# langtech-bsc/quantool

Measured on AMD Instinct MI355X. Metric: quantized weights/sec (GPTQ int4, Llama-3-8B, 512 calib samples), higher is better.
Workload: dtype f32

## Files before the change

include/quantool_amd.h:

```cpp
#ifndef QUANTOOL_AMD_H
#define QUANTOOL_AMD_H

#include <stddef.h>
#include <stdint.h>

#ifdef __cplusplus
extern "C" {
#endif

typedef void* qt_stream_t;

enum qt_status {
    QT_OK = 0,
    QT_ERR_INVALID = -1,
    QT_ERR_NOT_PD = -2,
    QT_ERR_WORKSPACE = -3,
    QT_ERR_HIP = -4,
    QT_ERR_UNSUPPORTED = -5
};

enum qt_dtype { QT_F32 = 0, QT_BF16 = 1, QT_F16 = 2 };

int qt_version(void);
const char* qt_last_error(void);
// ... 73 lines not shown
int qt_awq_weight_mean_accumulate(const void* W, int w_dtype, int R, int K, int64_t ldw, int group_size,
                                  float* w_sum, void* workspace, size_t workspace_bytes,
                                  qt_stream_t stream);
int qt_awq_scales(const float* x_abs_sum, int64_t n_tokens, const float* w_sum, int64_t n_rows, int K,
                  int n_grid, int duo_scaling, float* scales, qt_stream_t stream);
int qt_symmetrize_lower(float* G, int K, qt_stream_t stream);
size_t qt_awq_loss_workspace_bytes(int R, int K);
int qt_awq_loss(const void* W, int w_dtype, int R, int K, int64_t ldw, const float* s, int group_size,
                int symmetric, int num_bits, const float* Gfull, int64_t n_tokens, int exact, float weight,
                int accumulate, float* loss_out, void* workspace, size_t workspace_bytes, qt_stream_t stream);
size_t qt_awq_losses_workspace_bytes(int R, int K, int n_grid);
int qt_awq_losses(const void* W, int w_dtype, int R, int K, int64_t ldw, const float* scales, int n_grid,
                  int group_size, int symmetric, int num_bits, const float* Gfull, int64_t n_tokens, float weight,
                  int accumulate, float* losses, void* workspace, size_t workspace_bytes, qt_stream_t stream);
int qt_argmin_f32(const float* values, int n, int32_t* index_out, qt_stream_t stream);
int qt_awq_pseudo_quantize(const void* W, int w_dtype, int R, int K, int64_t ldw, const float* s, int group_size,
                           int symmetric, int num_bits, void* out, int64_t ldo, qt_stream_t stream);
int qt_scale_columns(const void* W, int w_dtype, int R, int K, int64_t ldw, const float* s, int divide,
                     void* out, int64_t ldo, qt_stream_t stream);
int qt_rtn_quantize(const void* W, int w_dtype, int R, int K, int64_t ldw, const float* scale,
                    const float* zp, int G, int group_size, int num_bits, int8_t* Qt, qt_stream_t stream);

size_t qt_col_absmax_workspace_bytes(int R, int K);
int qt_col_absmax_accumulate(const void* W, int w_dtype, int R, int K, int64_t ldw, float* wmax,
                             void* workspace, size_t workspace_bytes, qt_stream_t stream);
int qt_smoothquant_scales(const float* cmin, const float* cmax, const float* wmax, int K, float alpha,
                          float* s, qt_stream_t stream);

size_t qt_sgemm_tn_f32_workspace_bytes(int M, int N);
int qt_sgemm_tn_f32(const float* A, int64_t lda, const float* B, int64_t ldb, const float* Cin,
                    int64_t ldcin, float* Cout, int64_t ldcout, int M, int N, int kdim, int skip_zero_k,
                    int mode, int allow_split_k, void* workspace, size_t workspace_bytes, qt_stream_t stream);

int qt_xtx_tile_table_check(int K, int* n_tiles_out, int* chunk_panels_out, int* round_panels_out);

size_t qt_xtx_dot_workspace_bytes(int64_t n_tokens, int K);
int qt_xtx_dot(const void* X, int x_dtype, int64_t n_tokens, int K, int64_t ldx, const float* H, double scale,
               float* out, int accumulate, void* workspace, size_t workspace_bytes, qt_stream_t stream);

size_t qt_gemm3_tn_f32_workspace_bytes(int M, int N, int k);
int qt_gemm3_tn_f32(const float* A, int64_t lda, const float* B, int64_t ldb, float* C, int64_t ldc, int M,
                    int N, int k, int kind, void* workspace, size_t workspace_bytes, qt_stream_t stream);
int qt_gemm3_tn_f32_ex(const float* A, int64_t lda, const float* B, int64_t ldb, float* C, int64_t ldc, int M, int N,
                       int k, int kind, int tri, int tight, int batch, int64_t bsA, int64_t bsB, int64_t bsC,
                       void* workspace, size_t workspace_bytes, qt_stream_t stream);

int qt_gemm3_tn_f16x2(const float* A, int64_t lda, const float* B, int64_t ldb, float* C, int64_t ldc, int M, int N,
                      int k, int kind, int tri, int tight, int batch, int64_t bsA, int64_t bsB, int64_t bsC,
                      const float* bound_a, const float* bound_b, void* workspace, size_t workspace_bytes,
                      qt_stream_t stream);

int qt_gemm3_plan_check(int Tm, int Tn, int c_end, int tri, int* n_items_out, int* n_slabs_out, int* longest_out);
int qt_chol_g3_plan_check(int K, int merged, int min_chunks, long long* counts_out);
enum qt_act { QT_ACT_SILU = 0 };
#define QT_I8_MID_MAX_M 128
#define QT_I8_MID_K_UNIT 128
#define QT_I8_RING_K_UNIT 128
#define QT_I8_RING_SLOTS 8
#define QT_I8_RING_LEAD 6
#define QT_I8_RING_W4_K_UNIT 128
#define QT_I8_RING_W4_SLOTS 8
#define QT_I8_RING_W4_LEAD 6
#define QT_SPLITK_I8_K_UNIT 128
#define QT_SPLITK_I8_MAX_SPLITS 32
#define QT_SPLITK_I8_MIN_K_TILES 4
#define QT_MOE_I8_WIDE_K_UNIT 128
#define QT_MOE_I8_WIDE_TILE_ROWS 128
#define QT_MOE_I8_WIDE_MAX_E 4096
enum qt_weight_format { QT_W_INT8 = 0, QT_W_INT4_PACKED = 1 };
int qt_quantize_tokens_i8(const void* X, int x_dtype, int64_t M, int K, int64_t ldx, const int32_t* col_perm,
                          int symmetric, int8_t* Xq, float* s_x, int32_t* zp_x, qt_stream_t stream);
int qt_act_mul_quantize_i8(const void* gate, int64_t ldg, const void* up, int64_t ldu, int x_dtype, int64_t M, int K,
                           int act, const int32_t* col_perm, int symmetric, int8_t* Xq, float* s_x, int32_t* zp_x,
                           void* H, int64_t ldh, qt_stream_t stream);
int qt_rmsnorm_quantize_i8(const void* X, int64_t ldx, const void* weight, int x_dtype, int64_t M, int K, float eps,
                           const int32_t* col_perm, int symmetric, int8_t* Xq, float* s_x, int32_t* zp_x,
                           void* Y, int64_t ldy, float* rstd, qt_stream_t stream);
int qt_gemm_i8(const int8_t* Xq, int64_t M, int K, const void* Wq, int w_format, int N, const float* s_x,
               const int32_t* zp_x, const float* s_w, int G, const int32_t* wsum, const void* bias, void* Y,
               int out_dtype, int64_t ldy, qt_stream_t stream);
int qt_gemm_i8_skinny(const int8_t* Xq, int M, int K, const void* Wq, int w_format, int N, const float* s_x,
                      const int32_t* zp_x, const float* s_w, int G, const int32_t* wsum, const void* bias, void* Y,
                      int out_dtype, int64_t ldy, qt_stream_t stream);
int qt_gemm_i8_ring(const int8_t* Xq, int64_t M, int K, const void* Wq, int w_format, int N, const float* s_x,
                    const int32_t* zp_x, const float* s_w, int G, const int32_t* wsum, const void* bias, void* Y,
                    int out_dtype, int64_t ldy, qt_stream_t stream);
int qt_gemm_i8_ring_w4(const int8_t* Xq, int64_t M, int K, const void* Wq, int w_format, int N, const float* s_x,
                       const int32_t* zp_x, const float* s_w, int G, const int32_t* wsum, const void* bias, void* Y,
                       int out_dtype, int64_t ldy, qt_stream_t stream);
int qt_gemm_i8_mid(const int8_t* Xq, int64_t M, int K, const void* Wq, int w_format, int N, const float* s_x,
                   const int32_t* zp_x, const float* s_w, int G, const int32_t* wsum, const void* bias, void* Y,
                   int out_dtype, int64_t ldy, qt_stream_t stream);
int qt_splitk_gemm_i8_plan(int64_t M, int N, int K, int cus, int splits_requested, int* splits,
                           size_t* workspace_size);
int qt_splitk_gemm_i8_range(int k_tiles, int splits, int s, int* t0, int* t1);
int qt_splitk_gemm_i8(const int8_t* Xq, int64_t M, int K, const void* Wq, int w_format, int N, const float* s_x,
                      const int32_t* zp_x, const float* s_w, int G, const int32_t* wsum, const void* bias, void* Y,
                      int out_dtype, int64_t ldy, int splits, void* workspace, size_t workspace_size,
                      qt_stream_t stream);

int qt_moe_route(const void* top_k_index, int index_is_int64, int64_t T, int k, int E, int32_t* offsets,
                 int32_t* src_token, int32_t* src_slot, int32_t* row_of, qt_stream_t stream);
int qt_gemm_i8_grouped(const int8_t* Xq, int K, const int32_t* row_idx, int64_t R, const int32_t* offsets, int E,
                       const void* Wq, int w_format, int N, const float* s_x, const int32_t* zp_x, const float* s_w,
                       int G, const int32_t* wsum, void* Y, int out_dtype, int64_t ldy, qt_stream_t stream);
int qt_gemm_i8_skinny_grouped(const int8_t* Xq, int K, const int32_t* row_idx, int64_t R, const int32_t* offsets,
// ... 66 lines not shown
```

quantool_amd/csrc/cholesky.hip:

```cpp
#include <stdlib.h>
#include <string.h>

#include <map>
#include <tuple>
#include <vector>

#include "chol_layout.h"
#include "common.h"
#include "gemm3_tn.h"
#include "sgemm_tn.h"

namespace {

static_assert(CHOL_CHUNK_ROWS == G3_CHUNK_ROWS, "chol_layout.h counts k chunks as gemm3_tn.h cuts them");
static int chol_block_env(const char* name) {
    const char* e = getenv(name);
    if (!e) return 0;
    int x = atoi(e) / 128 * 128;
    return x < 128 ? 128 : (x > NBO_MAX ? NBO_MAX : x);
}
struct G3Step {
    int n_items = 0, n_red = 0;
    size_t item_off = 0, red_off = 0;
};
struct CholG3Plan {
    bool any = false;
    std::vector<G3Step> fac, inv;
    std::vector<G3Step> row;
    char* blob = nullptr;
    size_t blob_bytes = 0;
    int max_slabs = 0;
    bool any_row = false;
};

static int chol_g3_min_chunks() {
    const char* on = getenv("QT_CHOL_G3");
    if (on && atoi(on) == 0) return 0;
    const char* e = getenv("QT_CHOL_G3_MIN_CHUNKS");
    const int x = e ? atoi(e) : 64;
    return x < 1 ? 1 : x;
}

static int chol_g3_target_items(int K) {
    const char* e = getenv("QT_G3_TARGET_ITEMS");
    if (e && atoi(e) > 0) return atoi(e);
    return K < 8192 ? 96 : 256;
}

enum { CHOL_TWO_PHASE = 0, CHOL_WALK = 1, CHOL_WALK_MERGED = 2 };
static int chol_merge_mode() {
    const char* e = getenv("QT_CHOL_MERGE");
    if (!e) return CHOL_WALK_MERGED;
    if (strcmp(e, "order") == 0) return CHOL_WALK;
    return atoi(e) != 0 ? CHOL_WALK_MERGED : CHOL_TWO_PHASE;
}

static void chol_g3_build(int K, int NBO, int NBI, int min_chunks, int target_items, bool merged, CholG3Plan& pl,
// ... 445 lines not shown
        for (int r = 0; r < 16; ++r) zb[r] = 0.0f;
#pragma unroll
        for (int r = 0; r < 16; ++r) {
            const int k = (r & 3) + 8 * (r >> 2) + 4 * h;
            const float av = D32[(b * 32 + k) * 32 + l31];
            zb = __builtin_amdgcn_mfma_f32_32x32x2f32(av, acc[b][r], zb, 0, 0, 0);
        }
        acc[b] = zb;
#pragma unroll
        for (int a = b + 1; a < 4; ++a) {
#pragma unroll
            for (int r = 0; r < 16; ++r) {
                const int k = (r & 3) + 8 * (r >> 2) + 4 * h;
                const float av = -Rs[(32 * b + k) * NB + 32 * a + l31];
                acc[a] = __builtin_amdgcn_mfma_f32_32x32x2f32(av, zb[r], acc[a], 0, 0, 0);
            }
        }
    }
    float* Dinv = Dinv_all + (size_t)blk * NB * NB;
    float* Yd = Y + (size_t)(blk * NB) * ldy + blk * NB;
#pragma unroll
    for (int a = 0; a < 4; ++a)
#pragma unroll
        for (int r = 0; r < 16; ++r) {
            const int row = 32 * a + (r & 3) + 8 * (r >> 2) + 4 * h;
            const bool in = row < n && col < n;
            const float z = (in && row >= col) ? acc[a][r] : 0.0f;
            Dinv[col * NB + row] = z;
            if (in) Yd[(size_t)row * ldy + col] = z;
        }
}

__global__ __launch_bounds__(256) void transpose_lower_block_kernel(const float* __restrict__ Y, int64_t ldy, int w,
                                                                    float* __restrict__ XT, int ldx, int64_t bsY,
                                                                    int64_t bsXT) {
    if (blockIdx.z) {
        Y += (size_t)blockIdx.z * bsY;
        XT += (size_t)blockIdx.z * bsXT;
    }
    __shared__ float tile[32][33];
    const int bx = blockIdx.x * 32, by = blockIdx.y * 32;
    const int tx = threadIdx.x & 31, ty = threadIdx.x >> 5;
    for (int r = ty; r < 32; r += 8) {
        const int m = bx + r, k = by + tx;
        tile[r][tx] = (m < w && k < w && k <= m) ? Y[(size_t)m * ldy + k] : 0.0f;
    }
    __syncthreads();
    for (int r = ty; r < 32; r += 8) {
        const int k = by + r, m = bx + tx;
        if (k < w && m < w) XT[(size_t)k * ldx + m] = tile[tx][r];
    }
}

__global__ __launch_bounds__(256) void flat_reverse_lower_to_upper_kernel(float* __restrict__ U, int K, int64_t bsU) {
    U += (size_t)blockIdx.z * bsU;
    const int j = blockIdx.x * blockDim.x + threadIdx.x;
    const int i = blockIdx.y;
    if (j >= K || j < i) return;
    const size_t e = (size_t)i * K + j;
    const size_t pe = (size_t)(K - 1 - i) * K + (K - 1 - j);
    if (i == j) {
        if (e <= pe) {
            const float t = U[e];
            U[e] = U[pe];
            U[pe] = t;
        }
    } else {
        U[e] = U[pe];
        U[pe] = 0.0f;
    }
}

__global__ __launch_bounds__(256) void identity_if_failed_kernel(float* __restrict__ U, int K,
                                                                 const int32_t* __restrict__ info, int64_t bsU) {
    if (info[blockIdx.z] == 0) return;
    U += (size_t)blockIdx.z * bsU;
    for (int i = blockIdx.x; i < K; i += gridDim.x)
        for (int j = threadIdx.x; j < K; j += blockDim.x) U[(size_t)i * K + j] = (i == j) ? 1.0f : 0.0f;
}

__global__ __launch_bounds__(256) void chol_scales_kernel(const float* __restrict__ A, int64_t bsA, int K,
                                                          const float* __restrict__ min_eig_lb, int32_t* __restrict__ e,
                                                          int32_t* __restrict__ info) {
    __shared__ float red[256];
    const int b = blockIdx.x, nprob = gridDim.x;
    const float* Ab = A + (size_t)b * bsA;
    float m = 0.0f;
    for (int i = threadIdx.x; i < K; i += 256) m = fmaxf(m, Ab[(size_t)i * K + i]);
    red[threadIdx.x] = m;
    __syncthreads();
    for (int s = 128; s > 0; s >>= 1) {
        if ((int)threadIdx.x < s) red[threadIdx.x] = fmaxf(red[threadIdx.x], red[threadIdx.x + s]);
        __syncthreads();
    }
    if (threadIdx.x == 0) {
        auto clampe = [](float t) { return (int)fminf(fmaxf(t, (float)-G3_E_MAX), (float)G3_E_MAX); };
        const float d = red[0], lb = min_eig_lb[b];
        e[b] = (d > 0.0f && d < 3.0e38f) ? clampe(3.0f - ceilf(0.5f * log2f(d))) : 0;
        if (lb > 0.0f && lb < 3.0e38f) {
            e[nprob + b] = clampe(3.0f - ceilf(-0.5f * log2f(lb)));
        } else {
            e[nprob + b] = 0;
            info[b] = K + 1;
        }
    }
}

}


static CholLayout chol_layout(int K, const CholG3Plan* g3) { return CholLayout(K, g3->any, g3->max_slabs); }

extern "C" size_t qt_cholesky_inverse_upper_batched_workspace_bytes(int K, int n_problems) {
    if (K <= 0 || n_problems <= 0) return 0;
    int nbo_, nbi_;
    const CholG3Plan* g3 = chol_blocks(K, nbo_, nbi_);
    return chol_layout(K, g3).batch_bytes(n_problems, g3->blob_bytes);
}

extern "C" size_t qt_cholesky_inverse_upper_workspace_bytes(int K) {
    return qt_cholesky_inverse_upper_batched_workspace_bytes(K, 1);
}

constexpr size_t INV_LDS = (size_t)(NB * LDT + NB * LDP) * sizeof(float);
constexpr size_t POTF2_LDS = (size_t)(NB * LDA + 4 * 32 * 32) * sizeof(float);
constexpr size_t RD_LDS = RD_STRIDE * sizeof(float);

struct CholCtx {
    float *A, *Y;
    int K, nprob, NBO, NBI;
    int64_t sA, sY, sW;
    float *T, *TI, *XT, *Rd, *Dinv, *split_ws;
    size_t split_ws_bytes;
    unsigned short *Rpl, *Ypl;
    int64_t plane_stride;
    float* g3_slabs;
    char* g3_tab;
    const CholG3Plan* g3;
    const CholG3Plan* tab;
    int planes;
    int merge_mode;
    int32_t *info, *eR, *eY;
    int prio;
    hipStream_t stream;
};

static int chol_resolve(CholCtx& c, const float* min_eig_lb) {
    bool f16x2 = min_eig_lb != nullptr;
    if (const char* e = getenv("QT_CHOL_PLANES")) {
        if (strcmp(e, "bf16x3") == 0) f16x2 = false;
        else if (strcmp(e, "f16x2") == 0) {
            QT_CHECK_ARG(min_eig_lb, "qt_cholesky_inverse_upper: QT_CHOL_PLANES=f16x2 needs a bound on lambda_min (the _bounded entry points)");
        } else {
            QT_CHECK_ARG(false, "qt_cholesky_inverse_upper: QT_CHOL_PLANES=%s (bf16x3 | f16x2)", e);
        }
    }
    c.g3 = chol_blocks(c.K, c.NBO, c.NBI);
    c.planes = (f16x2 && c.g3->any) ? G3_F16X2 : G3_BF16X3;
    c.merge_mode = (c.g3->any && c.NBO == c.NBI) ? chol_merge_mode() : CHOL_TWO_PHASE;
    c.tab = c.g3;
    if (c.merge_mode == CHOL_WALK_MERGED) {
        c.tab = chol_g3_plan(c.K, c.NBO, c.NBI, true);
        if (!c.tab->any || !c.tab->any_row || c.tab->max_slabs > c.g3->max_slabs || c.tab->blob_bytes > c.g3->blob_bytes) {
            c.tab = c.g3;
            c.merge_mode = CHOL_TWO_PHASE;
        }
    }
    return QT_OK;
}

enum CholHome { IN_A, IN_Y, IN_WS };
struct CholOperand { float* p; int64_t ld; CholHome home; };
static int64_t chol_stride(const CholCtx& c, CholHome h) { return h == IN_A ? c.sA : h == IN_Y ? c.sY : c.sW; }

static SgemmArgs chol_sgemm_args(const CholCtx& c, CholOperand A, CholOperand B, CholOperand C, int M, int N, int kdim,
                                 int k_mode, int mode, bool offer_split) {
    SgemmArgs g;
    g.A = A.p; g.lda = A.ld;
    g.B = B.p; g.ldb = B.ld;
    g.Cin = mode == SG_MODE_SUB ? C.p : nullptr; g.ldcin = mode == SG_MODE_SUB ? C.ld : 0;
    g.Cout = C.p; g.ldcout = C.ld;
    g.M = M; g.N = N; g.kdim = kdim; g.k_mode = k_mode; g.mode = mode;
    g.split_ws = offer_split ? c.split_ws : nullptr; g.split_ws_bytes = offer_split ? c.split_ws_bytes : 0;
    g.batch = c.nprob;
    g.bsA = chol_stride(c, A.home); g.bsB = chol_stride(c, B.home); g.bsCin = g.bsCout = chol_stride(c, C.home);
    g.bs_split = c.sW;
    return g;
}

static int g3_row(const CholCtx& c, const G3Step& st, const unsigned short* Bplanes, int col_a0, int col_b0, int M, int N,
                  float* C, CholHome c_home, int mode, bool second = false) {
    G3Args a;
    a.Apl = c.Rpl; a.Bpl = Bplanes; a.plane_stride = c.plane_stride; a.ld = c.K;
    a.rowA0 = a.rowB0 = 0; a.colA0 = col_a0; a.colB0 = col_b0; a.colmax = c.K;
    a.M = M; a.N = N; a.C = C; a.ldc = c.K; a.mode = mode;
    a.slabs = c.g3_slabs;
    a.items = (const G3Item*)(c.g3_tab + st.item_off); a.n_items = st.n_items;
    a.red = (const G3Red*)(c.g3_tab + st.red_off); a.n_red = st.n_red;
    a.batch = c.nprob;
    a.bsApl = a.bsBpl = c.sW * 2;
    a.bsC = chol_stride(c, c_home); a.bsSlabs = c.sW;
    if (c.planes == G3_F16X2) {
        a.planes = G3_F16X2; a.eA = c.eR; a.eB = Bplanes == c.Rpl ? c.eR : c.eY;
    }
    if (second) {
        a.Bpl1 = c.Ypl; a.colB01 = 0; a.eB1 = c.eY;
        a.C1 = c.TI; a.ldc1 = c.K; a.bsC1 = c.sW; a.mode1 = G3_SET;
        a.N1 = col_a0;
// ... 35 lines not shown
        }
    }
    const int rem = K - J1;
    if (c.g3->any) {
        if (rem > 0) {
            float* RJ = A + (size_t)J0 * K + J0;
            unsigned short* pl = c.Rpl + (size_t)J0 * K + J0;
            int rc = c.planes == G3_F16X2
                         ? qt_split2h_launch(RJ, K, J1 - J0, K - J0, pl, K, c.plane_stride, 0, 0, 0, c.eR, c.stream, nprob, c.sA, c.sW * 2)
                         : qt_split3_launch(RJ, K, J1 - J0, K - J0, pl, K, c.plane_stride, 0, 0, 0, c.stream, nprob, c.sA, c.sW * 2);
            if (rc) return rc;
        }
    } else if (rem > 0) {
        const CholOperand RJ = {A + (size_t)J0 * K + J1, K, IN_A};
        SgemmArgs g = chol_sgemm_args(c, RJ, RJ, {A + (size_t)J1 * K + J1, K, IN_A}, rem, rem, J1 - J0, SG_K_FULL, SG_MODE_SUB, false);
        g.upper_only = 1;
        int rc = qt_sgemm_tn(g, c.stream);
        if (rc) return rc;
    }
    return QT_OK;
}

static int trinv(const CholCtx& c, int blk0, int n) {
    const char* e = getenv("QT_CHOL_TRINV");
    if (e && strcmp(e, "div") == 0)
        hipLaunchKernelGGL(trinv_batched_kernel, dim3(n, c.nprob), dim3(NB), INV_LDS, c.stream, (const float*)c.Rd, c.K, c.Dinv,
                           c.Y, (int64_t)c.K, c.sW, c.sY, blk0);
    else
        hipLaunchKernelGGL(trinv_mfma_kernel, dim3(n, c.nprob), dim3(256), RD_LDS, c.stream, (const float*)c.Rd, c.K, c.Dinv,
                           c.Y, (int64_t)c.K, c.sW, c.sY, blk0);
    QT_LAUNCH_CHECK();
    return QT_OK;
}

static int inv_product(const CholCtx& c, const BlockRow& I) {
    const int K = c.K, I0 = I.J0;
    if (I0 == 0) return QT_OK;
    if (c.g3->any && c.tab->inv[I.Jb].n_items > 0) return g3_row(c, c.tab->inv[I.Jb], c.Ypl, I0, 0, I.rows(), I0, c.TI, IN_WS, G3_SET);
    return qt_sgemm_tn(chol_sgemm_args(c, {c.A + I0, K, IN_A}, {c.Y, K, IN_Y}, {c.TI, K, IN_WS}, I.rows(), I0, I0, SG_K_FROM_N0,
                                       SG_MODE_SET, true),
                       c.stream);
}

static int split_row(const CholCtx& c, const BlockRow& I) {
    const int K = c.K, I0 = I.J0;
    if (!c.g3->any || I.J1 >= K) return QT_OK;
    if (c.planes == G3_F16X2)
        return qt_split2h_launch(c.Y + (size_t)I0 * K, K, I.rows(), I.J1, c.Ypl + (size_t)I0 * K, K, c.plane_stride, 1, I0, 0, c.eY,
                                 c.stream, c.nprob, c.sY, c.sW * 2);
    return qt_split3_launch(c.Y + (size_t)I0 * K, K, I.rows(), I.J1, c.Ypl + (size_t)I0 * K, K, c.plane_stride, 1, I0, 0, c.stream,
                            c.nprob, c.sY, c.sW * 2);
}

static int inv_row(const CholCtx& c, const BlockRow& I) {
    const int K = c.K, I0 = I.J0, I1 = I.J1, Wi = I.rows();
    float* Y = c.Y;
    for (int i0 = I0 + NB; i0 < I1; i0 += NB) {
        const int i = i0 / NB, nbi = (K - i0 < NB) ? K - i0 : NB;
        const CholOperand Yi = {Y + (size_t)i0 * K + I0, K, IN_Y}, Tp = {c.T, K, IN_WS};
        int rc = qt_sgemm_tn(chol_sgemm_args(c, {c.A + (size_t)I0 * K + i0, K, IN_A}, {Y + (size_t)I0 * K + I0, K, IN_Y}, Tp, nbi,
                                             i0 - I0, i0 - I0, SG_K_FROM_N0, SG_MODE_SET, false),
                             c.stream);
        if (rc) return rc;
        rc = qt_sgemm_tn(chol_sgemm_args(c, {c.Dinv + (size_t)i * NB * NB, NB, IN_WS}, Tp, Yi, nbi, i0 - I0, nbi, SG_K_FULL,
                                         SG_MODE_NEG, false),
                         c.stream);
        if (rc) return rc;
    }
    if (I0 == 0) return split_row(c, I);
    hipLaunchKernelGGL(transpose_lower_block_kernel, dim3((Wi + 31) / 32, (Wi + 31) / 32, c.nprob), dim3(256), 0, c.stream,
                       (const float*)(Y + (size_t)I0 * K + I0), (int64_t)K, Wi, c.XT, NBO_MAX, c.sY, c.sW);
    QT_LAUNCH_CHECK();
    int rc = qt_sgemm_tn(chol_sgemm_args(c, {c.XT, NBO_MAX, IN_WS}, {c.TI, K, IN_WS}, {Y + (size_t)I0 * K, K, IN_Y}, Wi, I0, Wi,
                                         SG_K_FULL, SG_MODE_NEG, false),
                         c.stream);
    if (rc) return rc;
    return split_row(c, I);
}

static int chol_run_two_phase(const CholCtx& c) {
    for (BlockRow J(c.K, c.NBO); J; ++J) {
        int rc = fac_product(c, J);
        if (!rc) rc = fac_panels(c, J);
        if (rc) return rc;
    }
    int rc = trinv(c, 0, (c.K + NB - 1) / NB);
    if (rc) return rc;
    for (BlockRow I(c.K, c.NBI); I; ++I) {
        rc = inv_product(c, I);
        if (!rc) rc = inv_row(c, I);
        if (rc) return rc;
    }
    return QT_OK;
}

static int chol_run_walk(const CholCtx& c) {
    for (BlockRow J(c.K, c.NBO); J; ++J) {
        int rc;
        if (c.merge_mode == CHOL_WALK_MERGED && c.tab->row[J.Jb].n_items > 0) {
            rc = g3_row(c, c.tab->row[J.Jb], c.Rpl, J.J0, J.J0, J.rows(), c.K - J.J0, c.A + (size_t)J.J0 * c.K + J.J0, IN_A, G3_SUB,
                        true);
        } else {
            rc = fac_product(c, J);
            if (!rc) rc = inv_product(c, J);
        }
        if (!rc) rc = fac_panels(c, J);
        if (!rc) rc = trinv(c, J.J0 / NB, (J.rows() + NB - 1) / NB);
        if (!rc) rc = inv_row(c, J);
        if (rc) return rc;
    }
    return QT_OK;
}

static hipError_t chol_lds_attrs() {
    static QtOncePerDevice lds_attr;
    return lds_attr.run([] {
        const auto attr = hipFuncAttributeMaxDynamicSharedMemorySize;
        hipError_t e = hipFuncSetAttribute((const void*)potf2_kernel, attr, (int)POTF2_LDS);
        if (e == hipSuccess) e = hipFuncSetAttribute((const void*)trsm_rt_kernel, attr, (int)RD_LDS);
        if (e == hipSuccess) e = hipFuncSetAttribute((const void*)trinv_batched_kernel, attr, (int)INV_LDS);
        if (e == hipSuccess) e = hipFuncSetAttribute((const void*)trinv_mfma_kernel, attr, (int)RD_LDS);
        return e;
    });
}

static int chol_run(float* A, int64_t strideA, int K, float* U, int64_t strideU, int32_t* info, int nprob, void* workspace,
                    size_t workspace_bytes, hipStream_t stream, const float* min_eig_lb = nullptr) {
    CholCtx c = {};
    c.A = A; c.Y = U; c.K = K; c.nprob = nprob; c.info = info; c.stream = stream;
    if (int rc = chol_resolve(c, min_eig_lb)) return rc;
    const CholLayout L = chol_layout(K, c.g3);
    const size_t need = L.batch_bytes(nprob, c.g3->blob_bytes);
    if (!workspace || workspace_bytes < need) {
        qt_set_error("qt_cholesky_inverse_upper: workspace %zu < required %zu", workspace_bytes, need);
        return QT_ERR_WORKSPACE;
    }
    char* ws = (char*)qt_align_up((size_t)workspace, 256);
    c.sW = (int64_t)(L.bytes() / 4); c.sA = nprob > 1 ? strideA : 0; c.sY = nprob > 1 ? strideU : 0;
    c.T = (float*)(ws + L.T); c.TI = (float*)(ws + L.TI); c.XT = (float*)(ws + L.XT);
    c.Rd = (float*)(ws + L.Rd); c.Dinv = (float*)(ws + L.Dinv);
    c.split_ws = (float*)(ws + L.split); c.split_ws_bytes = L.split_bytes;
    c.plane_stride = (int64_t)K * K;
    if (c.g3->any) {
        c.Rpl = (unsigned short*)(ws + L.Rpl); c.Ypl = (unsigned short*)(ws + L.Ypl);
        c.g3_slabs = (float*)(ws + L.slabs); c.g3_tab = ws + L.tables(nprob);
        QT_HIP(hipMemcpyAsync(c.g3_tab, c.tab->blob, c.tab->blob_bytes, hipMemcpyHostToDevice, stream));
    }
    static_assert(2 * SG_MAX_BATCH * sizeof(int32_t) <= (size_t)NB * NB * 2, "the exponents fit the smallest third plane");
    c.eR = c.planes == G3_F16X2 ? (int32_t*)(c.Rpl + 2 * c.plane_stride) : nullptr;
    c.eY = c.planes == G3_F16X2 ? c.eR + nprob : nullptr;
    QT_HIP(chol_lds_attrs());
    QT_HIP(hipMemsetAsync(info, 0, sizeof(int32_t) * nprob, stream));
    c.prio = qt_chain_prio();
    if (c.planes == G3_F16X2) {
        hipLaunchKernelGGL(chol_scales_kernel, dim3(nprob), dim3(256), 0, stream, (const float*)A, c.sA, K, min_eig_lb, c.eR, info);
        QT_LAUNCH_CHECK();
    }
    if (int rc = c.merge_mode == CHOL_TWO_PHASE ? chol_run_two_phase(c) : chol_run_walk(c)) return rc;
    hipLaunchKernelGGL(flat_reverse_lower_to_upper_kernel, dim3((K + 255) / 256, K, nprob), dim3(256), 0, stream, U, K, c.sY);
    QT_LAUNCH_CHECK();
    hipLaunchKernelGGL(identity_if_failed_kernel, dim3(K < 1024 ? K : 1024, 1, nprob), dim3(256), 0, stream, U, K,
                       (const int32_t*)info, c.sY);
    QT_LAUNCH_CHECK();
    return QT_OK;
}

static int chol_check_batch(const char* fn, bool ptrs, int K, int n_problems, int64_t strideA, int64_t strideU) {
    QT_CHECK_ARG(K > 0 && ptrs && n_problems >= 1 && n_problems <= SG_MAX_BATCH, "%s: bad arguments (1 <= n_problems <= %d)", fn,
                 SG_MAX_BATCH);
    QT_CHECK_ARG(n_problems == 1 || (strideA >= (int64_t)K * K && strideU >= (int64_t)K * K && strideA % 4 == 0 && strideU % 4 == 0),
                 "%s: strides must be multiples of 4 elements and >= K*K", fn);
    return QT_OK;
}

extern "C" int qt_cholesky_inverse_upper(float* A, int K, float* U, int32_t* info, void* workspace,
                                         size_t workspace_bytes, qt_stream_t stream_) {
    QT_CHECK_ARG(K > 0 && A && U && info, "qt_cholesky_inverse_upper: bad arguments");
    return chol_run(A, 0, K, U, 0, info, 1, workspace, workspace_bytes, (hipStream_t)stream_);
}

extern "C" int qt_cholesky_inverse_upper_batched(float* A, int64_t strideA, int K, float* U, int64_t strideU, int32_t* info,
                                                 int n_problems, void* workspace, size_t workspace_bytes,
                                                 qt_stream_t stream_) {
    if (int rc = chol_check_batch("qt_cholesky_inverse_upper_batched", A && U && info, K, n_problems, strideA, strideU)) return rc;
    return chol_run(A, strideA, K, U, strideU, info, n_problems, workspace, workspace_bytes, (hipStream_t)stream_);
}

extern "C" int qt_cholesky_inverse_upper_bounded(float* A, int K, float* U, int32_t* info, const float* min_eig_lb,
                                                 void* workspace, size_t workspace_bytes, qt_stream_t stream_) {
    QT_CHECK_ARG(K > 0 && A && U && info && min_eig_lb, "qt_cholesky_inverse_upper_bounded: bad arguments");
    return chol_run(A, 0, K, U, 0, info, 1, workspace, workspace_bytes, (hipStream_t)stream_, min_eig_lb);
}

extern "C" int qt_cholesky_inverse_upper_batched_bounded(float* A, int64_t strideA, int K, float* U, int64_t strideU,
                                                         int32_t* info, int n_problems, const float* min_eig_lb,
                                                         void* workspace, size_t workspace_bytes, qt_stream_t stream_) {
    if (int rc = chol_check_batch("qt_cholesky_inverse_upper_batched_bounded", A && U && info && min_eig_lb, K, n_problems,
                                  strideA, strideU))
        return rc;
    return chol_run(A, strideA, K, U, strideU, info, n_problems, workspace, workspace_bytes, (hipStream_t)stream_, min_eig_lb);
}

extern "C" int qt_chol_g3_plan_check(int K, int merged, int min_chunks, long long* counts_out) {
    if (K <= 0) return -1;
    constexpr int NBX = 512, TRI_STEP = 256 / G3_CHUNK_ROWS;
    if (min_chunks <= 0) min_chunks = 64;
    const int cap = chol_g3_target_items(K);
    CholG3Plan sep, pl;
    std::vector<char> sep_bytes, bytes;
    chol_g3_build(K, NBX, NBX, min_chunks, cap, false, sep, sep_bytes);
    chol_g3_build(K, NBX, NBX, min_chunks, cap, merged != 0, pl, bytes);
    if (pl.max_slabs > sep.max_slabs || pl.blob_bytes > sep.blob_bytes) return -2;
    long long launches = 0, n_items = 0, n_slabs = 0;
    auto check = [&](const G3Step& st, int Tm, int Tn0, int tri0, int Tn1, int c_end) -> int {
        if (st.n_items <= 0) return 0;
        const G3Item* items = (const G3Item*)(bytes.data() + st.item_off);
        const G3Red* red = (const G3Red*)(bytes.data() + st.red_off);
        if (st.n_items > cap && st.n_items > Tm * (Tn0 + Tn1)) return -3;
        const int Tn[2] = {Tn0, Tn1};
        auto lo_of = [&](int seg, int tj) { return (seg == 1 || tri0) ? TRI_STEP * tj : 0; };
        std::vector<int> cover((size_t)2 * Tm * (Tn0 + Tn1 + 1) * c_end, 0);
        auto cell = [&](int seg, int ti, int tj, int c) { return (((size_t)seg * Tm + ti) * (Tn0 + Tn1 + 1) + tj) * c_end + c; };
        std::vector<int> owner(sep.max_slabs, -1);
        int slabs_here = 0;
        for (int q = 0; q < st.n_items; ++q) {
            const G3Item& it = items[q];
            const int seg = (it.tile & G3_SEG_BIT) ? 1 : 0, ti = it.tile >> 16, tj = it.tile & G3_TJ_MASK;
            if (ti < 0 || ti >= Tm || tj >= Tn[seg]) return -4;
            const int lo = lo_of(seg, tj);
            if (it.c_lo < lo || it.c_hi > c_end || it.c_hi - it.c_lo < 2) return -5;
            for (int c = it.c_lo; c < it.c_hi; ++c) cover[cell(seg, ti, tj, c)]++;
            if (it.slab < 0) {
                if (it.c_lo != lo || it.c_hi != c_end) return -6;
            } else {
                if (it.slab >= sep.max_slabs) return -7;
                if (owner[it.slab] >= 0) return -8;
                owner[it.slab] = q;
                ++slabs_here;
            }
        }
        for (int seg = 0; seg < 2; ++seg)
            for (int ti = 0; ti < Tm; ++ti)
                for (int tj = 0; tj < Tn[seg]; ++tj)
                    for (int c = 0; c < c_end; ++c)
                        if (cover[cell(seg, ti, tj, c)] != (c >= lo_of(seg, tj) ? 1 : 0)) return -9;
        int in_red = 0;
        for (int r = 0; r < st.n_red; ++r) {
            const G3Red& e = red[r];
            if (e.count < 2 || e.first < 0 || e.first + e.count > sep.max_slabs || (e.seg != 0 && e.seg != 1)) return -10;
            const int want_tile = e.tile | (e.seg ? G3_SEG_BIT : 0);
            int prev_hi = lo_of(e.seg, e.tile & G3_TJ_MASK);
            for (int q = 0; q < e.count; ++q) {
                const int o = owner[e.first + q];
                if (o < 0 || items[o].tile != want_tile || items[o].c_lo != prev_hi) return -11;
// ... 34 lines not shown
```

quantool_amd/hip/_lib.py:

```python
from __future__ import annotations

import ctypes
from ctypes import c_char_p, c_double, c_float, c_int, c_int32, c_int64, c_size_t, c_void_p
from pathlib import Path

_PKG = Path(__file__).resolve().parent.parent
LIB_PATH = _PKG / "lib" / "libquantool_hip.so"

QT_OK = 0
QT_ERR_INVALID = -1
QT_ERR_NOT_PD = -2
QT_ERR_WORKSPACE = -3
QT_ERR_HIP = -4
QT_ERR_UNSUPPORTED = -5

QT_F32, QT_BF16, QT_F16 = 0, 1, 2
QT_W_INT8, QT_W_INT4_PACKED = 0, 1

SIGNATURES = {
    "qt_version": (c_int, []),
    "qt_last_error": (c_char_p, []),
    "qt_xtx_workspace_bytes": (c_size_t, [c_int64, c_int]),
    "qt_xtx_accumulate": (c_int, [c_void_p, c_int, c_int64, c_int, c_int64, c_void_p, c_void_p, c_size_t, c_void_p]),
    "qt_xtx_accumulate_batched": (c_int, [c_void_p, c_int, c_void_p, c_void_p, c_int, c_void_p, c_int, c_void_p, c_size_t,
# ... 10 lines not shown
    "qt_hessian_prepare_damp": (c_int, [c_void_p, c_int, c_int64, c_float, c_void_p, c_void_p, c_void_p, c_void_p,
                                        c_void_p, c_void_p, c_size_t, c_void_p]),
    "qt_hessian_diag": (c_int, [c_void_p, c_int, c_int64, c_void_p, c_void_p]),
    "qt_argsort_desc": (c_int, [c_void_p, c_int, c_void_p, c_void_p, c_void_p]),
    "qt_cholesky_inverse_upper_workspace_bytes": (c_size_t, [c_int]),
    "qt_cholesky_inverse_upper": (c_int, [c_void_p, c_int, c_void_p, c_void_p, c_void_p, c_size_t, c_void_p]),
    "qt_cholesky_inverse_upper_batched_workspace_bytes": (c_size_t, [c_int, c_int]),
    "qt_cholesky_inverse_upper_batched": (c_int, [c_void_p, c_int64, c_int, c_void_p, c_int64, c_void_p, c_int, c_void_p,
                                                  c_size_t, c_void_p]),
    "qt_cholesky_inverse_upper_bounded": (c_int, [c_void_p, c_int, c_void_p, c_void_p, c_void_p, c_void_p, c_size_t,
                                                  c_void_p]),
    "qt_cholesky_inverse_upper_batched_bounded": (c_int, [c_void_p, c_int64, c_int, c_void_p, c_int64, c_void_p, c_int,
                                                          c_void_p, c_void_p, c_size_t, c_void_p]),
    "qt_group_minmax_qparams": (c_int, [c_void_p, c_int, c_int, c_int, c_int64, c_int, c_int, c_int, c_void_p,
                                        c_void_p, c_void_p, c_void_p, c_void_p]),
    "qt_weight_gather_f32": (c_int, [c_void_p, c_int, c_int, c_int, c_int64, c_void_p, c_void_p, c_void_p,
                                     c_void_p]),
    "qt_weight_gather_qparams": (c_int, [c_void_p, c_int, c_int, c_int, c_int64, c_void_p, c_void_p, c_int, c_int, c_int,
                                         c_void_p, c_void_p, c_void_p, c_void_p, c_void_p, c_int64, c_void_p]),
    "qt_gptq_sweep_workspace_bytes": (c_size_t, [c_int, c_int, c_int]),
    "qt_gptq_sweep": (c_int, [c_void_p, c_int, c_int, c_void_p, c_void_p, c_void_p, c_int, c_void_p, c_int, c_int,
                              c_void_p, c_void_p, c_void_p, c_size_t, c_void_p]),
    "qt_gptq_sweep_grouped": (c_int, [c_void_p, c_int, c_int, c_void_p, c_int64, c_int, c_void_p, c_void_p, c_void_p, c_int,
                                      c_void_p, c_int, c_int, c_void_p, c_void_p, c_void_p, c_size_t, c_void_p]),
    "qt_pack_int4": (c_int, [c_void_p, c_int, c_int, c_void_p, c_void_p, c_void_p]),
    "qt_awq_weight_mean_workspace_bytes": (c_size_t, [c_int, c_int]),
    "qt_awq_weight_mean_accumulate": (c_int, [c_void_p, c_int, c_int, c_int, c_int64, c_int, c_void_p, c_void_p,
                                              c_size_t, c_void_p]),
    "qt_awq_scales": (c_int, [c_void_p, c_int64, c_void_p, c_int64, c_int, c_int, c_int, c_void_p, c_void_p]),
    "qt_symmetrize_lower": (c_int, [c_void_p, c_int, c_void_p]),
    "qt_awq_loss_workspace_bytes": (c_size_t, [c_int, c_int]),
    "qt_awq_loss": (c_int, [c_void_p, c_int, c_int, c_int, c_int64, c_void_p, c_int, c_int, c_int, c_void_p, c_int64,
                            c_int, c_float, c_int, c_void_p, c_void_p, c_size_t, c_void_p]),
    "qt_awq_losses_workspace_bytes": (c_size_t, [c_int, c_int, c_int]),
    "qt_awq_losses": (c_int, [c_void_p, c_int, c_int, c_int, c_int64, c_void_p, c_int, c_int, c_int, c_int, c_void_p,
                              c_int64, c_float, c_int, c_void_p, c_void_p, c_size_t, c_void_p]),
    "qt_argmin_f32": (c_int, [c_void_p, c_int, c_void_p, c_void_p]),
    "qt_awq_pseudo_quantize": (c_int, [c_void_p, c_int, c_int, c_int, c_int64, c_void_p, c_int, c_int, c_int, c_void_p,
                                       c_int64, c_void_p]),
    "qt_scale_columns": (c_int, [c_void_p, c_int, c_int, c_int, c_int64, c_void_p, c_int, c_void_p, c_int64,
                                 c_void_p]),
    "qt_rtn_quantize": (c_int, [c_void_p, c_int, c_int, c_int, c_int64, c_void_p, c_void_p, c_int, c_int, c_int,
                                c_void_p, c_void_p]),
    "qt_col_absmax_workspace_bytes": (c_size_t, [c_int, c_int]),
    "qt_col_absmax_accumulate": (c_int, [c_void_p, c_int, c_int, c_int, c_int64, c_void_p, c_void_p, c_size_t,
                                         c_void_p]),
    "qt_smoothquant_scales": (c_int, [c_void_p, c_void_p, c_void_p, c_int, c_float, c_void_p, c_void_p]),
    "qt_xtx_dot_workspace_bytes": (c_size_t, [c_int64, c_int]),
    "qt_xtx_dot": (c_int, [c_void_p, c_int, c_int64, c_int, c_int64, c_void_p, c_double, c_void_p, c_int, c_void_p,
                           c_size_t, c_void_p]),
    "qt_gemm3_plan_check": (c_int, [c_int, c_int, c_int, c_int, c_void_p, c_void_p, c_void_p]),
    "qt_xtx_tile_table_check": (c_int, [c_int, c_void_p, c_void_p, c_void_p]),
    "qt_chol_g3_plan_check": (c_int, [c_int, c_int, c_int, c_void_p]),
    "qt_gemm3_tn_f32_workspace_bytes": (c_size_t, [c_int, c_int, c_int]),
    "qt_gemm3_tn_f32": (c_int, [c_void_p, c_int64, c_void_p, c_int64, c_void_p, c_int64, c_int, c_int, c_int, c_int,
                                c_void_p, c_size_t, c_void_p]),
    "qt_gemm3_tn_f32_ex": (c_int, [c_void_p, c_int64, c_void_p, c_int64, c_void_p, c_int64, c_int, c_int, c_int, c_int,
                                   c_int, c_int, c_int, c_int64, c_int64, c_int64, c_void_p, c_size_t, c_void_p]),
    "qt_gemm3_tn_f16x2": (c_int, [c_void_p, c_int64, c_void_p, c_int64, c_void_p, c_int64, c_int, c_int, c_int, c_int,
                                  c_int, c_int, c_int, c_int64, c_int64, c_int64, c_void_p, c_void_p, c_void_p, c_size_t,
                                  c_void_p]),
    "qt_sgemm_tn_f32_workspace_bytes": (c_size_t, [c_int, c_int]),
    "qt_sgemm_tn_f32": (c_int, [c_void_p, c_int64, c_void_p, c_int64, c_void_p, c_int64, c_void_p, c_int64, c_int,
                                c_int, c_int, c_int, c_int, c_int, c_void_p, c_size_t, c_void_p]),
    "qt_profile_enable": (c_int, [c_int]),
    "qt_profile_read": (c_int, [c_int, c_void_p, c_void_p]),
    "qt_dequantize": (c_int, [c_void_p, c_int, c_int, c_void_p, c_void_p, c_void_p, c_int, c_void_p, c_void_p,
                              c_int, c_int64, c_void_p]),
    "qt_quantize_tokens_i8": (c_int, [c_void_p, c_int, c_int64, c_int, c_int64, c_void_p, c_int, c_void_p, c_void_p,
                                      c_void_p, c_void_p]),
    "qt_act_mul_quantize_i8": (c_int, [c_void_p, c_int64, c_void_p, c_int64, c_int, c_int64, c_int, c_int, c_void_p,
                                       c_int, c_void_p, c_void_p, c_void_p, c_void_p, c_int64, c_void_p]),
    "qt_rmsnorm_quantize_i8": (c_int, [c_void_p, c_int64, c_void_p, c_int, c_int64, c_int, c_float, c_void_p, c_int,
                                       c_void_p, c_void_p, c_void_p, c_void_p, c_int64, c_void_p, c_void_p]),
    "qt_gemm_i8": (c_int, [c_void_p, c_int64, c_int, c_void_p, c_int, c_int, c_void_p, c_void_p, c_void_p, c_int,
                           c_void_p, c_void_p, c_void_p, c_int, c_int64, c_void_p]),
    "qt_gemm_i8_skinny": (c_int, [c_void_p, c_int, c_int, c_void_p, c_int, c_int, c_void_p, c_void_p, c_void_p, c_int,
                                  c_void_p, c_void_p, c_void_p, c_int, c_int64, c_void_p]),
    "qt_gemm_i8_ring": (c_int, [c_void_p, c_int64, c_int, c_void_p, c_int, c_int, c_void_p, c_void_p, c_void_p, c_int,
                                c_void_p, c_void_p, c_void_p, c_int, c_int64, c_void_p]),
    "qt_gemm_i8_ring_w4": (c_int, [c_void_p, c_int64, c_int, c_void_p, c_int, c_int, c_void_p, c_void_p, c_void_p,
                                   c_int, c_void_p, c_void_p, c_void_p, c_int, c_int64, c_void_p]),
    "qt_gemm_i8_mid": (c_int, [c_void_p, c_int64, c_int, c_void_p, c_int, c_int, c_void_p, c_void_p, c_void_p, c_int,
                               c_void_p, c_void_p, c_void_p, c_int, c_int64, c_void_p]),
    "qt_splitk_gemm_i8_plan": (c_int, [c_int64, c_int, c_int, c_int, c_int, c_void_p, c_void_p]),
    "qt_splitk_gemm_i8_range": (c_int, [c_int, c_int, c_int, c_void_p, c_void_p]),
    "qt_splitk_gemm_i8": (c_int, [c_void_p, c_int64, c_int, c_void_p, c_int, c_int, c_void_p, c_void_p, c_void_p, c_int,
                                  c_void_p, c_void_p, c_void_p, c_int, c_int64, c_int, c_void_p, c_size_t, c_void_p]),
    "qt_gemm_i8_skinny_grouped": (c_int, [c_void_p, c_int, c_void_p, c_int64, c_void_p, c_int, c_void_p, c_int, c_int,
                                          c_void_p, c_void_p, c_void_p, c_int, c_void_p, c_void_p, c_int, c_int64,
                                          c_void_p]),
    "qt_moe_route": (c_int, [c_void_p, c_int, c_int64, c_int, c_int, c_void_p, c_void_p, c_void_p, c_void_p,
                             c_void_p]),
    "qt_gemm_i8_grouped": (c_int, [c_void_p, c_int, c_void_p, c_int64, c_void_p, c_int, c_void_p, c_int, c_int,
                                   c_void_p, c_void_p, c_void_p, c_int, c_void_p, c_void_p, c_int, c_int64, c_void_p]),
    "qt_gemm_i8_ring_grouped": (c_int, [c_void_p, c_int, c_void_p, c_int64, c_void_p, c_int, c_void_p, c_int, c_int,
                                        c_void_p, c_void_p, c_void_p, c_int, c_void_p, c_void_p, c_int, c_int64,
                                        c_int64, c_void_p]),
    "qt_moe_gemm_i8_ring_w4": (c_int, [c_void_p, c_int, c_void_p, c_int64, c_void_p, c_int, c_void_p, c_int, c_int,
                                       c_void_p, c_void_p, c_void_p, c_int, c_void_p, c_void_p, c_int, c_int64,
                                       c_int64, c_void_p]),
    "qt_moe_gemm_i8_wide": (c_int, [c_void_p, c_int, c_void_p, c_int64, c_void_p, c_int, c_void_p, c_int, c_int,
                                    c_void_p, c_void_p, c_void_p, c_int, c_void_p, c_void_p, c_int, c_int64,
                                    c_int64, c_void_p]),
    "qt_moe_combine": (c_int, [c_void_p, c_int, c_int, c_int64, c_void_p, c_void_p, c_int64, c_int, c_void_p,
                               c_void_p]),
# ... 56 lines not shown
```

Baseline: 3.234 billion.

## Fuse diagonal-block triangular inverse strip into one MFMA kernel

Adds yii_strip_kernel, which computes the within-block-row inverse Y_ii column strips in a single launch per block row. It uses MFMA 32x32x2 f32 with register-prefetched R/Dinv chunks and LDS-resident Y, and also writes the transposed XT tile. This replaces the per-NB-block loop of separate small launches plus a transpose kernel. The goal is to cut launch count and serialization in the Cholesky inverse used by GPTQ. The cost is a more complex kernel with large LDS use and limited parallelism, since there is only one workgroup per 32 columns. The new path is on by default, with QT_CHOL_YII=launches as fallback and a launch counter exposed for testing.

```diff
diff --git a/include/quantool_amd.h b/include/quantool_amd.h
--- a/include/quantool_amd.h
+++ b/include/quantool_amd.h
@@ -149,6 +149,7 @@
 
 int qt_gemm3_plan_check(int Tm, int Tn, int c_end, int tri, int* n_items_out, int* n_slabs_out, int* longest_out);
 int qt_chol_g3_plan_check(int K, int merged, int min_chunks, long long* counts_out);
+long long qt_chol_yii_fused_launches(void);
 enum qt_act { QT_ACT_SILU = 0 };
 #define QT_I8_MID_MAX_M 128
 #define QT_I8_MID_K_UNIT 128
diff --git a/quantool_amd/csrc/cholesky.hip b/quantool_amd/csrc/cholesky.hip
--- a/quantool_amd/csrc/cholesky.hip
+++ b/quantool_amd/csrc/cholesky.hip
@@ -1,8 +1,10 @@
 #include <stdlib.h>
 #include <string.h>
 
+#include <atomic>
 #include <map>
 #include <tuple>
+#include <type_traits>
 #include <vector>
 
 #include "chol_layout.h"
@@ -554,6 +556,130 @@
     }
 }
 
+constexpr int YII_COLS = 32, YII_LDY = YII_COLS + 1;
+constexpr int YII_KC = 64;
+constexpr size_t yii_lds_bytes(int Wi) { return ((size_t)NB * YII_COLS + (size_t)((Wi + NB - 1) / NB * NB) * YII_LDY) * sizeof(float); }
+
+__global__ __launch_bounds__(256) void yii_strip_kernel(const float* __restrict__ R, float* Y, int64_t ld, int Wi,
+                                                        const float* __restrict__ Dinv, float* __restrict__ XT, int ldx,
+                                                        int write_xt, int prio, int64_t bsA, int64_t bsY, int64_t bsW) {
+    qt_set_chain_prio(prio);
+    if (blockIdx.y) {
+        R += (size_t)blockIdx.y * bsA;
+        Y += (size_t)blockIdx.y * bsY;
+        Dinv += (size_t)blockIdx.y * bsW;
+        XT += (size_t)blockIdx.y * bsW;
+    }
+    extern __shared__ __attribute__((aligned(16))) float sm[];
+    float* Ts = sm;
+    float* Ys = sm + NB * YII_COLS;
+    const int tid = threadIdx.x, lane = tid & 63;
+    const int wave = __builtin_amdgcn_readfirstlane(tid >> 6);
+    const int l31 = lane & 31, h = lane >> 5;
+    const int s = blockIdx.x * YII_COLS;
+    const int jb = s / NB, nblk = (Wi + NB - 1) / NB;
+    const int m = 32 * wave + l31;
+
+    constexpr int CU = YII_KC / 2;
+    int li = jb + 1, lq = 0;
+    auto load_next = [&](float (&dst)[CU]) {
+        const bool past = li >= nblk;
+        const int i = past ? jb : li, nr = 2 * (i - jb);
+        const int nbi = (Wi - i * NB < NB) ? Wi - i * NB : NB;
+        const bool is_d = past || lq >= nr;
+        const int qd = past ? 0 : lq - nr;
+        const float* p = is_d ? Dinv + (size_t)i * NB * NB + (size_t)(YII_KC * qd + h) * NB + m
+                              : R + (size_t)(jb * NB + YII_KC * lq + h) * ld + i * NB + (m < nbi ? m : 0);
+        const int64_t pitch = is_d ? 2 * NB : 2 * ld;
+#pragma unroll
+        for (int u = 0; u < CU; ++u) dst[u] = p[(size_t)u * pitch];
+        const bool last = !past && lq == nr + 1;
+        li += last ? 1 : 0;
+        lq = (past || last) ? 0 : lq + 1;
+    };
+    float c0[CU], c1[CU], c2[CU];
+    load_next(c0);
+    load_next(c1);
+
+    {
+        const int c = tid & 31, r0 = tid >> 5;
+        const bool cok = s + c < Wi;
+        float v[16];
+#pragma unroll
+        for (int u = 0; u < 16; ++u) {
+            const int k = jb * NB + r0 + 8 * u;
+            const bool ok = cok && k < Wi;
+            v[u] = Y[(size_t)(ok ? k : s) * ld + (cok ? s + c : s)];
+        }
+        __builtin_amdgcn_sched_barrier(0);
+#pragma unroll
+        for (int u = 0; u < 16; ++u) {
+            const int k = jb * NB + r0 + 8 * u;
+            Ys[k * YII_LDY + c] = (cok && k < Wi) ? v[u] : 0.0f;
+        }
+    }
+    __syncthreads();
+
+    auto xt_block = [&](int mb) {
+        const int mm = mb * NB + (tid & 127);
+#pragma unroll
+        for (int u = 0; u < 16; ++u) {
+            const int c = (tid >> 7) + 2 * u, n = s + c;
+            if (n < Wi && mm < Wi) XT[(size_t)n * ldx + mm] = (mb >= jb && mm >= n) ? Ys[mm * YII_LDY + c] : 0.0f;
+        }
+    };
+    if (write_xt)
+        for (int mb = 0; mb <= jb; ++mb) xt_block(mb);
+
+    int pi = jb + 1, pq = 0;
+    f32x16 acc;
+#pragma unroll
+    for (int r = 0; r < 16; ++r) acc[r] = 0.0f;
+    auto do_chunk = [&](const float (&cur)[CU], float (&dst)[CU]) {
+        const int nr = 2 * (pi - jb), i0 = pi * NB, nbi = (Wi - i0 < NB) ? Wi - i0 : NB;
+        if (pq == nr) {
+#pragma unroll
+            for (int r = 0; r < 16; ++r) {
+                const int row = 32 * wave + (r & 3) + 8 * (r >> 2) + 4 * h;
+                Ts[row * YII_COLS + l31] = row < nbi ? acc[r] : 0.0f;
+                acc[r] = 0.0f;
+            }
+            __syncthreads();
+        }
+        load_next(dst);
+        __builtin_amdgcn_sched_barrier(0);
+        const float* B = pq < nr ? Ys + (jb * NB + YII_KC * pq + h) * YII_LDY + l31 : Ts + (YII_KC * (pq - nr) + h) * YII_COLS + l31;
+        const int ldb2 = pq < nr ? 2 * YII_LDY : 2 * YII_COLS;
+#pragma unroll
+        for (int u = 0; u < CU; ++u) acc = __builtin_amdgcn_mfma_f32_32x32x2f32(cur[u], B[u * ldb2], acc, 0, 0, 0);
+        if (pq == nr + 1) {
+#pragma unroll
+            for (int r = 0; r < 16; ++r) {
+                const int row = 32 * wave + (r & 3) + 8 * (r >> 2) + 4 * h;
+                if (row < nbi) {
+                    const float v = -acc[r];
+                    Y[(size_t)(i0 + row) * ld + s + l31] = v;
+                    Ys[(i0 + row) * YII_LDY + l31] = v;
+                }
+                acc[r] = 0.0f;
+            }
+            __syncthreads();
+            if (write_xt) xt_block(pi);
+            ++pi;
+            pq = 0;
+        } else {
+            ++pq;
+        }
+    };
+    while (pi < nblk) {
+        do_chunk(c0, c2);
+        if (pi >= nblk) break;
+        do_chunk(c1, c0);
+        if (pi >= nblk) break;
+        do_chunk(c2, c1);
+    }
+}
+
 __global__ __launch_bounds__(256) void flat_reverse_lower_to_upper_kernel(float* __restrict__ U, int K, int64_t bsU) {
     U += (size_t)blockIdx.z * bsU;
     const int j = blockIdx.x * blockDim.x + threadIdx.x;
@@ -642,10 +768,14 @@
     const CholG3Plan* tab;
     int planes;
     int merge_mode;
+    int yii_mode;
     int32_t *info, *eR, *eY;
     int prio;
     hipStream_t stream;
 };
+
+enum { CHOL_YII_LAUNCHES = 0, CHOL_YII_FUSED = 1 };
+static std::atomic<long long> yii_fused_launches{0};
 
 static int chol_resolve(CholCtx& c, const float* min_eig_lb) {
     bool f16x2 = min_eig_lb != nullptr;
@@ -656,6 +786,11 @@
         } else {
             QT_CHECK_ARG(false, "qt_cholesky_inverse_upper: QT_CHOL_PLANES=%s (bf16x3 | f16x2)", e);
         }
+    }
+    c.yii_mode = CHOL_YII_FUSED;
+    if (const char* e = getenv("QT_CHOL_YII")) {
+        if (strcmp(e, "launches") == 0) c.yii_mode = CHOL_YII_LAUNCHES;
+        else QT_CHECK_ARG(strcmp(e, "fused") == 0, "qt_cholesky_inverse_upper: QT_CHOL_YII=%s (launches | fused)", e);
     }
     c.g3 = chol_blocks(c.K, c.NBO, c.NBI);
     c.planes = (f16x2 && c.g3->any) ? G3_F16X2 : G3_BF16X3;
@@ -797,7 +932,7 @@
                             c.nprob, c.sY, c.sW * 2);
 }
 
-static int inv_row(const CholCtx& c, const BlockRow& I) {
+static int yii_launches(const CholCtx& c, const BlockRow& I) {
     const int K = c.K, I0 = I.J0, I1 = I.J1, Wi = I.rows();
     float* Y = c.Y;
     for (int i0 = I0 + NB; i0 < I1; i0 += NB) {
@@ -812,13 +947,32 @@
                          c.stream);
         if (rc) return rc;
     }
-    if (I0 == 0) return split_row(c, I);
+    if (I0 == 0) return QT_OK;
     hipLaunchKernelGGL(transpose_lower_block_kernel, dim3((Wi + 31) / 32, (Wi + 31) / 32, c.nprob), dim3(256), 0, c.stream,
                        (const float*)(Y + (size_t)I0 * K + I0), (int64_t)K, Wi, c.XT, NBO_MAX, c.sY, c.sW);
     QT_LAUNCH_CHECK();
-    int rc = qt_sgemm_tn(chol_sgemm_args(c, {c.XT, NBO_MAX, IN_WS}, {c.TI, K, IN_WS}, {Y + (size_t)I0 * K, K, IN_Y}, Wi, I0, Wi,
-                                         SG_K_FULL, SG_MODE_NEG, false),
-                         c.stream);
+    return QT_OK;
+}
+
+static int yii_fused(const CholCtx& c, const BlockRow& I) {
+    const int K = c.K, I0 = I.J0, Wi = I.rows();
+    const size_t at = (size_t)I0 * K + I0;
+    hipLaunchKernelGGL(yii_strip_kernel, dim3((Wi + YII_COLS - 1) / YII_COLS, c.nprob), dim3(256), yii_lds_bytes(Wi), c.stream,
+                       (const float*)(c.A + at), c.Y + at, (int64_t)K, Wi, (const float*)(c.Dinv + (size_t)(I0 / NB) * NB * NB), c.XT,
+                       NBO_MAX, I0 > 0 ? 1 : 0, c.prio, c.sA, c.sY, c.sW);
+    QT_LAUNCH_CHECK();
+    yii_fused_launches.fetch_add(1, std::memory_order_relaxed);
+    return QT_OK;
+}
+
+static int inv_row(const CholCtx& c, const BlockRow& I) {
+    const int K = c.K, I0 = I.J0, Wi = I.rows();
+    int rc = (c.yii_mode == CHOL_YII_FUSED && Wi > NB) ? yii_fused(c, I) : yii_launches(c, I);
+    if (rc) return rc;
+    if (I0 == 0) return split_row(c, I);
+    rc = qt_sgemm_tn(chol_sgemm_args(c, {c.XT, NBO_MAX, IN_WS}, {c.TI, K, IN_WS}, {c.Y + (size_t)I0 * K, K, IN_Y}, Wi, I0, Wi,
+                                     SG_K_FULL, SG_MODE_NEG, false),
+                     c.stream);
     if (rc) return rc;
     return split_row(c, I);
 }
@@ -865,6 +1019,7 @@
         if (e == hipSuccess) e = hipFuncSetAttribute((const void*)trsm_rt_kernel, attr, (int)RD_LDS);
         if (e == hipSuccess) e = hipFuncSetAttribute((const void*)trinv_batched_kernel, attr, (int)INV_LDS);
         if (e == hipSuccess) e = hipFuncSetAttribute((const void*)trinv_mfma_kernel, attr, (int)RD_LDS);
+        if (e == hipSuccess) e = hipFuncSetAttribute((const void*)yii_strip_kernel, attr, (int)yii_lds_bytes(NBO_MAX));
         return e;
     });
 }
@@ -945,6 +1100,8 @@
         return rc;
     return chol_run(A, strideA, K, U, strideU, info, n_problems, workspace, workspace_bytes, (hipStream_t)stream_, min_eig_lb);
 }
+
+extern "C" long long qt_chol_yii_fused_launches(void) { return yii_fused_launches.load(std::memory_order_relaxed); }
 
 extern "C" int qt_chol_g3_plan_check(int K, int merged, int min_chunks, long long* counts_out) {
     if (K <= 0) return -1;
diff --git a/quantool_amd/hip/_lib.py b/quantool_amd/hip/_lib.py
--- a/quantool_amd/hip/_lib.py
+++ b/quantool_amd/hip/_lib.py
@@ -86,6 +86,7 @@
     "qt_gemm3_plan_check": (c_int, [c_int, c_int, c_int, c_int, c_void_p, c_void_p, c_void_p]),
     "qt_xtx_tile_table_check": (c_int, [c_int, c_void_p, c_void_p, c_void_p]),
     "qt_chol_g3_plan_check": (c_int, [c_int, c_int, c_int, c_void_p]),
+    "qt_chol_yii_fused_launches": (ctypes.c_longlong, []),
     "qt_gemm3_tn_f32_workspace_bytes": (c_size_t, [c_int, c_int, c_int]),
     "qt_gemm3_tn_f32": (c_int, [c_void_p, c_int64, c_void_p, c_int64, c_void_p, c_int64, c_int, c_int, c_int, c_int,
                                 c_void_p, c_size_t, c_void_p]),
```

Result: no change. 3.251 billion, median of 6 (+0.5%).
